# danieleschmidt/grid-fed-rl-gym

Hardware: AMD Instinct MI355X
Metric: env steps/sec (batched feeders) (higher is better)
Workload: dtype f64

## Files before the change

grid_fed_rl_gym_amd/csrc/abi_debug.hip:

```cpp
#include <cstdlib>
#include <cstring>
#include <string>
#include <vector>

#include "handle.h"
#include "mesh_schedule.h"

using namespace gsi;

extern "C" {

int gs_mesh_schedule_dump(const gs_topology* topo, int32_t zero_z_mode, int32_t nw, int32_t ni, int32_t acc_cap, int32_t unit_budget, int32_t region_base,
                          int32_t slot_bytes, int32_t* header, char* why, int32_t why_cap, void* items, int32_t* rowinfo,
                          int32_t* adj_off, double* adj_y) {
  if (!topo || !header) return fail(nullptr, GS_E_INVALID, "topology / header is NULL");
  if (topo->struct_size != (int32_t)sizeof(gs_topology)) return fail(nullptr, GS_E_INVALID, "struct_size mismatch");
  if (nw < 1 || ni < 1 || acc_cap < 1) return fail(nullptr, GS_E_INVALID, "bad arguments");
  HostTopology ht;
  const std::string err = gs_compile_topology(*topo, zero_z_mode, false, true, ht);
  if (!err.empty()) return fail(nullptr, GS_E_INVALID, "topology: %s", err.c_str());
  MeshSchedule S;
  gs_mesh_schedule(ht, nw, ni, 8, region_base, slot_bytes, acc_cap, unit_budget, S);
  const int32_t hd[16] = {S.ok ? 1 : 0, S.n_levels, S.n_rows, S.max_rows_per_wave, S.n_pivots, S.msg_units, S.n_messages, S.n_accumulators,
                          S.max_degree, S.unit_bytes, S.zero_off, S.dummy_off, S.body_off, S.region_bytes, (int32_t)sizeof(GsMeshItem), (int32_t)S.adj_off.size()};
// ... 18 lines not shown
  gs_mesh_schedule(ht, nw, ni, 8, region_base, slot_bytes, acc_cap, unit_budget, S);
  if (!S.ok) return fail(nullptr, GS_E_TOPOLOGY, "%s", S.why.c_str());
  counts[0] = S.n_pairs; counts[1] = (int32_t)S.ytab.size(); counts[2] = (int32_t)S.adj_ent.size(); counts[3] = GS_MESH_WORDS;
  if (packed) memcpy(packed, S.packed.data(), S.packed.size() * sizeof(int32_t));
  if (rowinfo) memcpy(rowinfo, S.rowinfo_packed.data(), S.rowinfo_packed.size() * sizeof(int32_t));
  if (ytab) memcpy(ytab, S.ytab.data(), S.ytab.size() * sizeof(double));
  if (adj_ent) memcpy(adj_ent, S.adj_ent.data(), S.adj_ent.size() * sizeof(int32_t));
  return GS_OK;
}

int gs_flat_newton_map_dump(const gs_topology* topo, int32_t zero_z_mode, double* out) {
  if (!topo || !out) return fail(nullptr, GS_E_INVALID, "topology / out is NULL");
  if (topo->struct_size != (int32_t)sizeof(gs_topology)) return fail(nullptr, GS_E_INVALID, "struct_size mismatch");
  HostTopology ht;
  const std::string err = gs_compile_topology(*topo, zero_z_mode, false, true, ht);
  if (!err.empty()) return fail(nullptr, GS_E_INVALID, "topology: %s", err.c_str());
  for (int i = 0; i < ht.n; ++i)
    if (i != ht.slack && !(ht.th_free[i] && ht.vm_free[i])) return fail(nullptr, GS_E_TOPOLOGY, "a bus other than the slack is not a PQ bus");
  const int na = ht.n - 1, N2 = 2 * na, K = na + 1, tiles = (N2 + 15) / 16, steps = (K + 3) / 4;
  std::vector<double> wt;
  if (!flat_newton_map(ht, tiles, steps, wt)) return fail(nullptr, GS_E_TOPOLOGY, "the flat-start Jacobian is singular");
  for (int u = 0; u < N2; ++u)
    for (int k = 0; k < K; ++k) out[(size_t)u * K + k] = wt[((size_t)(u / 16) * steps + k / 4) * 64 + (u % 16) + 16 * (k % 4)];
  return GS_OK;
}

int gs_debug_stamps(gs_handle* h, uint64_t* cycles_out, int32_t n) {
  if (!h || !cycles_out || n < 1 || n > 16) return fail(h, GS_E_INVALID, "bad arguments");
  GS_ENTER(h);
  HIPCHK(h, hipStreamSynchronize(h->stream));
  if (!h->d_stamps) {
    int rc = dev_alloc(h, &h->d_stamps, 16 + 2 * GS_STAMP_BLOCKS);
    if (rc) return rc;
    HIPCHK(h, hipMemset(h->d_stamps, 0, (16 + 2 * GS_STAMP_BLOCKS) * sizeof(unsigned long long)));
    h->SC.stamps = h->d_stamps;
    h->DA.stamps = h->d_stamps;
    h->SA.stamps = h->d_stamps;
    h->SC.stamp_wave = getenv("GS_STAMP_WAVE") ? atoi(getenv("GS_STAMP_WAVE")) : 0;
    h->SC.block_times = getenv("GS_STAMP_BLOCK_TIMES") ? 1 : 0;
    for (int k = 0; k < n; ++k) cycles_out[k] = 0;
    return GS_OK;
  }
  unsigned long long tmp[16];
  HIPCHK(h, hipMemcpy(tmp, h->d_stamps, sizeof tmp, hipMemcpyDeviceToHost));
  HIPCHK(h, hipMemset(h->d_stamps, 0, sizeof tmp));
  for (int k = 0; k < n; ++k) cycles_out[k] = tmp[k];
// ... 104 lines not shown
```

grid_fed_rl_gym_amd/csrc/gridstep_abi.hip:

```cpp
#include <hip/hip_runtime.h>

#include <algorithm>
#include <cmath>
#include <cstdarg>
#include <cstdio>
#include <cstdlib>
#include <cstring>
#include <string>
#include <vector>

#include "handle.h"

using namespace gsi;

namespace {

thread_local std::string g_last_error;

int launch_pack(gs_handle* h, const int32_t* map, int C, double* dst) {
  if (C <= 0) return GS_OK;
  LaunchTimer lt(h, GS_K_PACK);
  dim3 grid(h->groups, (C + 63) / 64);
  hipLaunchKernelGGL(gs_k_pack, grid, dim3(256), 0, h->stream, map, h->d_cst, C, h->R.total, h->slab, dst, h->B);
  HIPCHK(h, hipGetLastError());
// ... 387 lines not shown
  UP(lu_orig_pos, lu_orig_pos);
  if ((rc = dev_upload(h, &T.lu_a_ptr, h->lu_a_ptr)) || (rc = dev_upload(h, &T.lu_a, h->lu_a)) || (rc = dev_upload(h, &T.lu_b_ptr, h->lu_b_ptr)) ||
      (rc = dev_upload(h, &T.lu_b, h->lu_b)) || (rc = dev_upload(h, &T.lu_c_ptr, h->lu_c_ptr)) || (rc = dev_upload(h, &T.lu_c, h->lu_c)) ||
      (rc = dev_upload(h, &T.lu_r_ptr, h->lu_r_ptr)) || (rc = dev_upload(h, &T.lu_r, h->lu_r))) return bail(rc);
  UP(dn_th_idx, dn_th_idx); UP(dn_vm_idx, dn_vm_idx);
  UP(bl_ptr, bl_ptr); UP(bl_idx, bl_idx); UP(bg_ptr, bg_ptr); UP(bg_idx, bg_idx); UP(bb_ptr, bb_ptr); UP(bb_idx, bb_idx);
  UP(load_base, load_base); UP(load_q, load_q); UP(gen_kind, gen_kind); UP(gen_cap, gen_cap); UP(gen_p0, gen_p0);
  UP(gen_p1, gen_p1); UP(gen_p2, gen_p2); UP(bat_cap, bat_cap); UP(bat_rating, bat_rating); UP(bat_eff, bat_eff);
#undef UP
  if (h->solve == SolveMember::nr_dense_mfma) {
    GsDenseArgs& D = h->DA;
    if ((rc = dev_upload(h, &D.act_bus, h->act_bus)) || (rc = dev_upload(h, &D.act_of, h->act_of)) || (rc = dev_upload(h, &D.ent_ptr, h->ent_ptr)) ||
        (rc = dev_upload(h, &D.ent, h->ent)) || (rc = dev_upload(h, &D.bent_ptr, h->bent_ptr)) || (rc = dev_upload(h, &D.bent, h->bent))) return bail(rc);
    D.row_ptr = T.row_ptr; D.col = T.col; D.G = T.G; D.Bv = T.Bv; D.Gd = T.Gd; D.Bd = T.Bd;
    D.th_free = T.th_free; D.vm_free = T.vm_free; D.fixed_v = T.fixed_v; D.v_set = T.v_set;
    const size_t blocks = (size_t)D.NB * D.NB * 64 * 64;
    if ((rc = dev_alloc(h, &D.scratch, (size_t)h->dense_grid * blocks)) || (h->dense_flat && (rc = dev_alloc(h, &D.flat, blocks + 8))) ||
        (!h->jinv_t.empty() && (rc = dev_upload(h, &D.jinv_t, h->jinv_t)))) return bail(rc);
  }
  if (h->step == StepMember::nr_mesh2 &&
      ((rc = dev_upload(h, &h->F2.mesh_items, h->mesh_items)) || (rc = dev_upload(h, &h->F2.mesh_rowinfo, h->mesh_rowinfo)))) return bail(rc);
  if (h->second_gen() &&
      ((rc = dev_upload(h, &h->F2.recs, h->f2recs)) || (rc = dev_upload(h, &h->F2.anc, h->f2anc)) || (rc = dev_upload(h, &h->F2.zbus, h->f2z)) ||
       (h->fs_slot.size() > 1 && ((rc = dev_upload(h, &h->F2.fixed_slot, h->fs_slot)) || (rc = dev_upload(h, &h->F2.fixed_val, h->fs_val)))))) return bail(rc);
  if (h->pz) {
    GsLineParamArgs& A = h->LP;
    const size_t Bm = (size_t)h->B * h->m;
    h->inst_r.assign(topo->line_r_inst, topo->line_r_inst + Bm); h->inst_x.assign(topo->line_x_inst, topo->line_x_inst + Bm);
    A.B = h->B; A.groups = h->groups; A.n_slots = ht.n + 3; A.m = ht.m; A.newton = h->f2().newton() ? 1 : 0;
    A.lyr_nom = T.lyr; A.lyi_nom = T.lyi;
    double *dr = nullptr, *dx = nullptr, *dpz = nullptr;
    const size_t n_pz = (size_t)h->groups * GS_PZ_NQ(A.n_slots, A.m) * GS_LANES * 2;
    if ((rc = dev_upload(h, &A.zero_z, h->pz_zero)) || (rc = dev_upload(h, &A.ops_ptr, h->pz_ops_ptr)) || (rc = dev_upload(h, &A.ops, h->pz_ops)) ||
        (rc = dev_upload(h, &A.has, h->pz_has)) || (rc = dev_alloc(h, &dr, Bm)) || (rc = dev_alloc(h, &dx, Bm)) ||
        (rc = dev_alloc(h, &h->d_pzmask, (size_t)h->B)) || (rc = dev_alloc(h, &dpz, n_pz))) return bail(rc);
    A.r = dr; A.x = dx; A.pz = dpz;
    if (hipMemcpy(dr, h->inst_r.data(), Bm * sizeof(double), hipMemcpyHostToDevice) != hipSuccess ||
        hipMemcpy(dx, h->inst_x.data(), Bm * sizeof(double), hipMemcpyHostToDevice) != hipSuccess ||
        hipMemset(dpz, 0, n_pz * sizeof(double)) != hipSuccess || hipDeviceSynchronize() != hipSuccess)
      return bail(fail(nullptr, GS_E_HIP, "per-instance line impedances: upload failed"));
    if ((rc = launch_line_params(h, nullptr))) return bail(fail(nullptr, rc, "%s", h->err.c_str()));
  }
  if (h->pl) {
    GsLoadParamArgs& A = h->LL;
    const size_t Bl = (size_t)h->B * h->n_loads;
    h->inst_load.assign(topo->load_base_inst, topo->load_base_inst + Bl);
// ... 455 lines not shown
```

grid_fed_rl_gym_amd/csrc/gs_internal.h:

```cpp
#pragma once
#include <stdint.h>

#if defined(GS_BUILD_EXPERIMENTS)
#define GS_EXPERIMENT_ENV(name) getenv(name)
#else
#define GS_EXPERIMENT_ENV(name) ((const char*)nullptr)
#endif

#define GS_LANES 64
#define GS_ELEM(row, lane) ((((size_t)(row) >> 1) << 7) + ((size_t)(lane) << 1) + ((size_t)(row) & 1))
#define GS_MAX_WAVES 16
#define GS_ELL_K 4

#if defined(__HIP_DEVICE_COMPILE__)
#define GS_CONST __attribute__((address_space(4)))
#else
#define GS_CONST
#endif

#define GS_ARGS_IN_PLACE(Block, name)                                                                                           \
  const __attribute__((address_space(4))) char* ka_ = (const __attribute__((address_space(4))) char*)__builtin_amdgcn_kernarg_segment_ptr(); \
  asm volatile("" : "+s"(ka_));                                                                                                \
  const Block* name = (const Block*)ka_

// ... 250 lines not shown
  unsigned long long* stamps;
  GsRows R;
};

struct GsPackArgs {
  const int32_t* map;
  const double* cst;
  double* out;
  int32_t obs_dim, tiles_per_pass;
  int32_t early_pass0, pair_ok;
  int32_t skip0, skip1;
  int32_t lean, pad0;
};

#define GS_F2_PITCH 33
#define GS_F2_CHILDREN 8
struct GsF2Rec {
  int32_t bus, parent, flags, last;
  int32_t nl, l0, l1, ng;
  int32_t g0, g1, nb, b0;
  int32_t b1, level, pad1, pad2;
  double zr, zi, yr, yi;
};
#define GS_MESH_ACC 4
struct GsMeshItem {
  int32_t vk_off, vj_off;
  int32_t xk_off, xj_off;
  int32_t flags;
  int32_t cq_off;
  int32_t adj_ptr, bus;
  double ykj_g, ykj_b, ykk_g, ykk_b;
  int32_t mout[8];
  int32_t cq_in[GS_MESH_ACC], rw_in[GS_MESH_ACC], cl_in[GS_MESH_ACC];
  int32_t nbr, pos;
  int32_t pad[10];
};
enum {
  GS_MESH_F_PIVOT = 1,
  GS_MESH_F_NBR = 2,
  GS_MESH_F_SLACKPOS = 4,
  GS_MESH_F_HV0_SHIFT = 4,
  GS_MESH_F_T_SHIFT = 8,
  GS_MESH_F_G_SHIFT = 12,
  GS_MESH_F_RMW_SHIFT = 16
};

// ... 8 lines not shown
  GS_MESH_WORDS = 16
};
#define GS_MESH_F_NADJ_SHIFT 24

struct GsF2Tables {
  const GsF2Rec* recs;
  const int32_t* anc;
  const double* zbus;
  int32_t n_slots;
  int32_t slack;
  int32_t n_jump;
  int32_t n_levels, pos_off, n_anc_ints, wg_offset;
  int32_t off_tile, off_anc, off_z, off_env, off_red, off_atom, lds_bytes;
  int32_t off_prof, ring_zero;
  int32_t env_genp, env_curt, env_batp, env_soc;
  int32_t n_fixed, fixed_slot0;
  double fixed_val0;
  const int32_t* fixed_slot; const double* fixed_val;
  double* nrflat; int32_t nrflat_mode, pad_nrflat;
  const int32_t* mesh_items; const int32_t* mesh_rowinfo;
  int32_t off_scr, mesh_nz;
  int32_t mesh_pairs, mesh_off_p;
  const double* mesh_w; int32_t mesh_w_steps, mesh_slack;
};

struct GsRolloutPostArgs {
  double* rew; uint8_t* done;
  double* obs_next;
  const int32_t* map; const double* cst;
  int32_t* term_count; int32_t* term_idx; double* term_obs; int32_t term_cap;
  int32_t obs_dim, t, B;
};

struct GsRolloutStep {
  double* rew; uint8_t* done;
  double* obs_prev;
  const int32_t* map; const double* cst;
  int32_t* term_count; int32_t* term_idx; double* term_obs;
  int32_t term_cap, obs_dim, t, active;
};

#define GS_STAMP_BLOCKS 2048
struct GsSolveCfg {
  double tolerance, alpha;
  int32_t max_iterations, jacobian_exact;
  unsigned long long* stamps;
// ... 69 lines not shown
```

grid_fed_rl_gym_amd/csrc/kernels_flow2.hip:

```cpp
#include <hip/hip_runtime.h>
#include <math.h>
#include <limits.h>
#include <type_traits>
#include <utility>

#include "../../include/gridstep.h"
#include "gs_internal.h"
#include "kernels.h"
#include "members.h"

#define ROW(r) S[(size_t)(r) * GS_LANES]
#include "env_device.h"

#pragma clang fp contract(off)

extern __shared__ __attribute__((aligned(16))) char f2_lds[];

__device__ __forceinline__ void f2_sync() { asm volatile("s_waitcnt vmcnt(0) lgkmcnt(0)\n\ts_barrier" ::: "memory"); }
__device__ __forceinline__ void f2_lds_sync() { asm volatile("s_waitcnt lgkmcnt(0)\n\ts_barrier" ::: "memory"); }

#define F2_AS3 __attribute__((address_space(3)))
#define F2_P(type, off) ((type F2_AS3*)((F2_AS3 char*)f2_lds + (off)))
#define F2_VP(type, off) ((volatile type F2_AS3*)((F2_AS3 char*)f2_lds + (off)))
typedef double f2_v2 __attribute__((ext_vector_type(2)));
// ... 106 lines not shown
  if (!st.done) {
    st.mm = mm; st.iters = it + 1;
    if (!(mm < INFINITY)) { st.status = GS_STATUS_NAN; st.done = true; }
    else if (crit < tol) { st.conv = 1; st.status = GS_STATUS_OK; st.done = true; }
  }
}
#define F2_SUM_SCALE 0x1p44
__device__ __forceinline__ unsigned long long f2_fix(double s) {
  const double d = __builtin_fma(fmin(s, 255.0), F2_SUM_SCALE, 0x1p52);
  return __builtin_bit_cast(unsigned long long, d) & 0x000fffffffffffffull;
}
__device__ __forceinline__ unsigned long long f2_fix_tolerance(double tol) {
  const double t = fmin(fmax(tol, 0.0), 255.0) * (0.5 * F2_SUM_SCALE);
  return (unsigned long long)t;
}
__device__ __forceinline__ void f2_check_sum(F2State& st, double mm, unsigned long long sum_fix, unsigned long long tol_fix, int it) {
  if (!st.done) {
    st.mm = mm; st.iters = it + 1;
    if (!(mm < INFINITY)) { st.status = GS_STATUS_NAN; st.done = true; }
    else if (sum_fix < tol_fix) { st.conv = 1; st.status = GS_STATUS_OK; st.done = true; }
  }
}

__device__ __forceinline__ double f2_angle(double f, double e) {
  if (!__all(e > 0.0 && fabs(f) <= 0.125 * e)) return atan2(f, e);
  const double t = f / e, z = t * t;
  double p = -1.0 / 19.0;
  p = __builtin_fma(p, z, 1.0 / 17.0); p = __builtin_fma(p, z, -1.0 / 15.0); p = __builtin_fma(p, z, 1.0 / 13.0);
  p = __builtin_fma(p, z, -1.0 / 11.0); p = __builtin_fma(p, z, 1.0 / 9.0); p = __builtin_fma(p, z, -1.0 / 7.0);
  p = __builtin_fma(p, z, 1.0 / 5.0); p = __builtin_fma(p, z, -1.0 / 3.0);
  return __builtin_fma(t * z, p, t);
}

__device__ const double kF2Series[16] = {-1.0 / 355687428096000.0, 1.0 / 1307674368000.0, -1.0 / 6227020800.0, 1.0 / 39916800.0, -1.0 / 362880.0,
                                         1.0 / 5040.0, -1.0 / 120.0, 1.0 / 6.0,
                                         1.0 / 20922789888000.0, -1.0 / 87178291200.0, 1.0 / 479001600.0, -1.0 / 3628800.0, 1.0 / 40320.0,
                                         -1.0 / 720.0, 1.0 / 24.0, -0.5};
enum { F2_ST_PROLOGUE = 0, F2_ST_INIT, F2_ST_MISMATCH, F2_ST_BOTTOM_UP, F2_ST_FLAG, F2_ST_TOP_DOWN, F2_ST_FINAL_MISMATCH, F2_ST_EPILOGUE,
       F2_ST_PRO_SCALAR, F2_ST_PRO_SPARE, F2_ST_EPI_BUSES, F2_ST_EPI_LINES, F2_ST_EPI_REDUCE, F2_ST_EPI_SCALARS };
struct F2Stamp {
  unsigned long long* p; unsigned long long t; bool mine;
  __device__ __forceinline__ void hit(int k) {
    if (p == nullptr) return;
    const unsigned long long now = __builtin_readcyclecounter();
    if (mine) p[k] += now - t;
    t = now;
  }
};

template <int SOLVER, int CHK, int NW, int NI, int IW, int PZ = 0, int PL = 0>
__device__ __forceinline__ void f2_step(const GsTables& T, const GsF2Tables& F, const GsRows& R, const GsSolveCfg& C, const GsEnvCfg& E,
                                        double* __restrict__ slab, int B, const double* __restrict__ actions, double total_load,
                                        const GsPackArgs& PA, const GsFusedChecks& FC, const GsRolloutStep& RS,
                                        const double* __restrict__ pz = nullptr, const double* __restrict__ pl = nullptr) {
  f2_touch_arguments();
  constexpr int HV = 64 / IW;
  constexpr unsigned SB = (unsigned)(IW + 1) * 16u;
  const int lane = threadIdx.x & 63, l = lane & (IW - 1), hv = lane / IW;
  auto f2_slot = [](int slot, int ll) -> unsigned { return __umul24((unsigned)slot, SB) + ((unsigned)ll << 4); };
  const int wave = __builtin_amdgcn_readfirstlane(threadIdx.x >> 6);
  const int bid = (int)blockIdx.x + F.wg_offset;
  const int g = bid / HV, hs = bid % HV, L = hs * IW + l;
  const int b = g * GS_LANES + L;
  const bool valid = b < B;
  const GsLaneRows S = gs_lane_rows(slab, g, R.total, L);
  const double* const pz_lane = PZ ? pz + ((size_t)g * GS_PZ_NQ(F.n_slots, T.m) * GS_LANES + L) * 2 : nullptr;
  auto pz_at = [&](int q) -> double2 { return *(const double2*)(pz_lane + (size_t)q * (2 * GS_LANES)); };
  const double* const pl_lane = PL ? pl + ((size_t)g * GS_PL_NQ(T.n_loads) * GS_LANES + L) * 2 : nullptr;
  auto pl_at = [&](int q) -> double2 { return *(const double2*)(pl_lane + (size_t)q * (2 * GS_LANES)); };
  int n = T.n, m = T.m, nsl = F.n_slots;
  int o_env = F.off_env, o_tile = F.off_tile, o_red = F.off_red, o_atom = F.off_atom, o_anc = F.off_anc, o_z = F.off_z, o_prof = F.off_prof;
  int n_tab = SOLVER == F2_FBS ? F.n_jump * nsl * 4 : F.n_anc_ints;
  const int32_t* anc_g = F.anc; const double* zbus_g = F.zbus;
// ... 1025 lines not shown
    auto publish = [&]() {
#pragma unroll
      for (int j = 0; j < NI; ++j) f2_st2(bufA + f2_slot(ibus[j], l), make_double2(sr[j], si[j]));
    };
    const bool cap = it + 1 >= C.max_iterations;
    if (!cap) {
      unsigned long long sum;
      const double mm = wg_max_sum(lmax, lsum, sum);
      stp.hit(F2_ST_FLAG);
      f2_check_sum(st, mm, sum, tol_fix, it + 1);
    }
    if (cap || __all(st.done)) { publish(); break; }
    if (!st.done) {
#pragma unroll
      for (int j = 0; j < NI; ++j) {
        const double rd = f2_rcp(__builtin_fma(sr[j], sr[j], si[j] * si[j]));
        IR[j] = (Pj[j] * sr[j]) * rd; II[j] = (Pj[j] * si[j]) * rd;
      }
    }
    backward([]() -> bool { return false; });
    stp.hit(F2_ST_BOTTOM_UP);
  }
  }
  f2_sync();
  stp.hit(F2_ST_FINAL_MISMATCH);

  const bool flat_lane = st.done && st.iters <= 1, any_flat = __any(flat_lane);
  auto final_ef = [&](int bus) -> double2 {
    double2 v = f2_ld2(f2_slot(bus, l));
    if (any_flat) { const double fv = T.fixed_v[bus] ? T.v_set[bus] : 1.0; if (flat_lane) v = make_double2(fv, 0.0); }
    return v;
  };
  double totloss0 = 0.0, f_old = 0.0, viol0 = 0.0, step0 = 0.0, eprew0 = 0.0;
  if (wave == 0) { totloss0 = ROW(R.TOTLOSS); f_old = ROW(R.FREQ); viol0 = ROW(R.VIOL); eprew0 = ROW(R.EPREW); step0 = valid ? kold + 1.0 : kold; }
  const bool chk = CHK && FC.enabled;
  if (chk && wave == 0 && hv == 0) { cell[l] = 0ull; cell[IW + l] = 0ull; }
  const GsChecksCfg& K = FC.C;
  double* Pv = chk ? FC.prev + (size_t)g * (n + 1) * GS_LANES + L : nullptr;
  constexpr int BUS_PASSES = CHK ? NI + 1 : 1;
  double pvp[BUS_PASSES];
  double pv_f = 0.0;
  int ck_has_prev = 0, ck_consec = 0, ck_emode = 0;
  if constexpr (CHK) {
    if (chk) {
#pragma unroll
      for (int q = 0; q < BUS_PASSES; ++q) { const int i0 = wave * HV + hv + q * HV * NW; pvp[q] = i0 < n ? Pv[(size_t)i0 * GS_LANES] : 0.0; }
      if (wave == 0) pv_f = Pv[(size_t)n * GS_LANES];
      if (wave == 0 && hv == 0 && b < (int)FC.Bp && valid) { ck_has_prev = FC.state[b]; ck_consec = FC.state[FC.Bp + b]; ck_emode = FC.state[2 * FC.Bp + b]; }
    }
  }
  int k_nlow = 0, k_nhigh = 0, k_mhigh = 0, k_mlow = 0, k_mem = 0, k_cover = 0, k_mover = 0, k_vbad = 0, k_fbad = 0;
  double k_dv = 0.0, k_ql = 0.0; int k_dvnan = 0, k_qlnan = 0;

  int over = 0;
  for (int k0 = wave * HV + hv; k0 < ((m + HV * NW - 1) / (HV * NW)) * (HV * NW); k0 += HV * NW) {
    const bool on = k0 < m; const int k = on ? k0 : m - 1;
    const int li = T.lfrom[k], lj = T.lto[k];
    double yr, yi;
    if constexpr (PZ != 0) { const double2 y = pz_at(2 * nsl + k); yr = y.x; yi = y.y; } else { yr = T.lyr[k]; yi = T.lyi[k]; }
    const double rating = T.lrating[k], rinv = T.lrating_inv[k];
    const double2 vi = final_ef(li), vj = final_ef(lj);
    const double dr = vi.x - vj.x, di = vi.y - vj.y;
    const double ir = __builtin_fma(yr, dr, -(yi * di)), ii = __builtin_fma(yr, di, yi * dr);
    const double sr = __builtin_fma(vi.x, ir, vi.y * ii), si = __builtin_fma(vi.y, ir, -(vi.x * ii));
    const double ql = (rating > 0.0) ? gs_div_by(sqrt(__builtin_fma(sr, sr, si * si)), rating, rinv) : 0.0;
    const double ld = (rating > 0.0) ? gs_div_by(fabs(sr), rating, rinv) : 0.0;
    if (on) {
      f2_row(S, R.LOAD + k) = ql;
      if (!PA.lean) f2_pair(S, R.FLOW + k) = make_double2(sr, ld);
      f2_st2(o_tile + (unsigned)k * SB + ((unsigned)l << 4), make_double2(sr, ld));
      over += (ld > 0.8) ? 1 : 0;
      if (chk) {
        const double cld_ = K.stride_cload == 2 ? ld : ql;
        const bool co = cld_ > K.c_load, mo = cld_ > K.m_load;
        k_cover += co; k_mover += mo;
        if (ql != ql) k_qlnan = 1; else k_ql = fmax(k_ql, ql);
        if (!(fabs(sr) < INFINITY)) k_fbad = 1;
        if (FC.line_mask) FC.line_mask[((size_t)g * m + k) * GS_LANES + L] = (uint8_t)(co | (mo << 1));
      }
    }
  }
  stp.hit(F2_ST_EPI_LINES);
  f2_lds_sync();
  double dev = 0.0, vmax = -INFINITY, vmin = INFINITY;
  int vflags = 0;
  auto bus_pass = [&](int i0, double pv) {
    const bool on = i0 < n; const int i = on ? i0 : n - 1;
    double2 ef = final_ef(i);
    if (!on) ef = make_double2(1.0, 0.0);
    const double v = sqrt(__builtin_fma(ef.x, ef.x, ef.y * ef.y));
    const double ang = f2_angle(ef.y, ef.x);
    if (on) {
      f2_st2(f2_slot(i, l), make_double2(v, ang));
      if (!PA.lean) f2_pair(S, R.VM + i) = make_double2(v, ang);
      dev += fabs(v - 1.0);
      vmax = fmax(vmax, v); vmin = fmin(vmin, v);
      vflags |= (v > E.v_max) ? 1 : 0;
      vflags |= (v < E.v_min) ? 2 : 0;
      if (chk) {
        const bool cl = v < K.c_vlo, ch = !cl && v > K.c_vhi;
        const bool mh = v > K.m_vhi, ml = v < K.m_vlo;
        const bool em = v > K.m_evhi || v < K.m_evlo;
        k_nlow += cl; k_nhigh += ch; k_mhigh += mh; k_mlow += ml; k_mem += em;
        const double d = fabs(v - pv);
        if (d != d) k_dvnan = 1; else k_dv = fmax(k_dv, d);
        Pv[(size_t)i * GS_LANES] = v;
        if (!(fabs(v) < INFINITY)) k_vbad = 1;
        if (FC.bus_mask) FC.bus_mask[((size_t)g * n + i) * GS_LANES + L] = (uint8_t)(cl | (ch << 1) | (ml << 2) | (mh << 3) | (em << 4));
      }
    }
  };
  const int bus_passes = (n + HV * NW - 1) / (HV * NW);
  if constexpr (CHK) {
    if (chk) {
#pragma unroll
      for (int q = 0; q < BUS_PASSES; ++q) { if (q < bus_passes) bus_pass(wave * HV + hv + q * HV * NW, pvp[q]); }
    } else {
      for (int i0 = wave * HV + hv; i0 < bus_passes * (HV * NW); i0 += HV * NW) bus_pass(i0, 0.0);
    }
  } else {
    for (int i0 = wave * HV + hv; i0 < bus_passes * (HV * NW); i0 += HV * NW) {
      const bool on = i0 < n; const int i = on ? i0 : n - 1;
      double2 ef = final_ef(i);
      if (!on) ef = make_double2(1.0, 0.0);
      const double v = sqrt(__builtin_fma(ef.x, ef.x, ef.y * ef.y));
      const double ang = f2_angle(ef.y, ef.x);
      if (on) {
        f2_st2(f2_slot(i, l), make_double2(v, ang));
        if (!PA.lean) f2_pair(S, R.VM + i) = make_double2(v, ang);
        dev += fabs(v - 1.0);
        vmax = fmax(vmax, v); vmin = fmin(vmin, v);
        vflags |= (v > E.v_max) ? 1 : 0;
        vflags |= (v < E.v_min) ? 2 : 0;
      }
    }
  }
  stp.hit(F2_ST_EPI_BUSES);
  {
    const double ls2 = f2_xsum<IW>(psum, l), dv2 = f2_xsum<IW>(dev, l);
    if (hv == 0) { red_lsum[wave * IW + l] = ls2; red_dev[wave * IW + l] = dv2; }
    if (vmax == vmax && vmax > -INFINITY) atomicMax(cell + 3 * IW + l, f2_bits(vmax));
    if (vmin == vmin && vmin < INFINITY) atomicMin(cell + 4 * IW + l, f2_bits(vmin));
    if (over) atomicAdd(icell + 0 * IW + l, (unsigned)over);
    if (vflags) atomicOr(icell + 1 * IW + l, (unsigned)vflags);
    if (chk) {
      if (k_nlow) atomicAdd(icell + 2 * IW + l, (unsigned)k_nlow);
      if (k_nhigh) atomicAdd(icell + 3 * IW + l, (unsigned)k_nhigh);
      if (k_mhigh) atomicAdd(icell + 4 * IW + l, (unsigned)k_mhigh);
      if (k_mlow) atomicAdd(icell + 5 * IW + l, (unsigned)k_mlow);
      if (k_mem) atomicAdd(icell + 6 * IW + l, (unsigned)k_mem);
      if (k_cover) atomicAdd(icell + 7 * IW + l, (unsigned)k_cover);
      if (k_mover) atomicAdd(icell + 8 * IW + l, (unsigned)k_mover);
      const unsigned fl = (unsigned)(k_vbad | (k_fbad << 1) | (k_dvnan << 2) | (k_qlnan << 3));
      if (fl) atomicOr(icell + 9 * IW + l, fl);
      atomicMax(cell + 0 * IW + l, f2_bits(k_dv));
      atomicMax(cell + 1 * IW + l, f2_bits(k_ql));
    }
  }
  f2_lds_sync();
// ... 125 lines not shown
    if (st.mm > K.q_tol * 100.0) q *= 0.6;
    if (st.iters <= 5) q *= 1.1; else if (st.iters > 20) q *= 0.9;
    q = fmin(q, 1.0);
    if (!st.conv || vbad || fbad) q = 0.0;
    OF(GS_CF_QUALITY) = q;
#undef OI
#undef OF
  }
  stp.hit(F2_ST_EPI_SCALARS);
  if (C.stamps && C.block_times && lane == 0 && bid < GS_STAMP_BLOCKS)
    atomicMax(&C.stamps[17 + 2 * bid], (unsigned long long)__builtin_amdgcn_s_memrealtime());
}

template <StepMember M> constexpr GsStepKernels f2_kernels() { return {}; }
#define F2_PTR_0(p) nullptr
#define F2_PTR_1(p) p
#define F2_KERNEL(kernel, name, CHK, PZ, PL, OCC)                                                                           \
  extern "C" __global__ void __launch_bounds__(64 * step_row(StepMember::name).nw) OCC                                      \
  kernel(GsTables T, GsF2Tables F, GsRows R, GsSolveCfg C, GsEnvCfg E, double* __restrict__ slab, int B,                     \
         const double* __restrict__ actions, double total_load, GsPackArgs PA, GsFusedChecks FC, GsRolloutStep RS,          \
         const double* __restrict__ pz, const double* __restrict__ pl) {                                                    \
    constexpr StepMemberRow r = step_row(StepMember::name);                                                                 \
    GS_ARGS_IN_PLACE(F2ArgBlock, A);                                                                                        \
    f2_step<r.solver, CHK, r.nw, r.ni, r.iw, PZ, PL>(A->T, A->F, A->R, A->C, A->E, A->slab, A->B, A->actions, A->total_load, A->PA, \
                                                   A->FC, A->RS, F2_PTR_##PZ(pz), F2_PTR_##PL(pl));                         \
  }
#define F2_FORM(name, suffix, PZ, PL, OCC)                                                                                  \
  F2_KERNEL(gs_k_step_##name##suffix, name, 0, PZ, PL, OCC)                                                                 \
  F2_KERNEL(gs_k_stepc_##name##suffix, name, 1, PZ, PL, OCC)
#define F2_FNS(name, suffix) {gs_k_step_##name##suffix, gs_k_stepc_##name##suffix}
#define F2_MEMBER_NO_PZ(name, OCC)                                                                                          \
  F2_FORM(name, , 0, 0, OCC)                                                                                                \
  F2_FORM(name, _pl, 0, 1, OCC)                                                                                             \
  template <> constexpr GsStepKernels f2_kernels<StepMember::name>() { return {{{F2_FNS(name, ), F2_FNS(name, _pl)}, {}}}; }
#define F2_MEMBER(name, OCC)                                                                                                \
  F2_FORM(name, , 0, 0, OCC)                                                                                                \
  F2_FORM(name, _pl, 0, 1, OCC)                                                                                             \
  F2_FORM(name, _pz, 1, 0, OCC)                                                                                             \
  F2_FORM(name, _pz_pl, 1, 1, OCC)                                                                                          \
  template <> constexpr GsStepKernels f2_kernels<StepMember::name>() {                                                      \
    return {{{F2_FNS(name, ), F2_FNS(name, _pl)}, {F2_FNS(name, _pz), F2_FNS(name, _pz_pl)}}};                              \
  }

#if defined(GS_BUILD_EXPERIMENTS)
F2_MEMBER_NO_PZ(fbs_flow2, )
#endif
F2_MEMBER(nr_flow2, )
// ... 107 lines not shown
```

grid_fed_rl_gym_amd/csrc/members.h:

```cpp
#pragma once
#include <cstddef>

enum class SolveMember { nr_tree, nr_sparse_lu, fbs, nr_dense_pivot, nr_tree_lds, fbs_lds, fbs_flow, nr_dense_mfma, nr_sparse_lds };

enum class StepMember {
  none, fbs_flow2s, fbs_flow2h, fbs_flow2x,
#if defined(GS_BUILD_EXPERIMENTS)
  fbs_flow2,
#endif
  nr_flow2s, nr_flow2, nr_mesh2
};
constexpr int kStepMemberCount = (int)StepMember::nr_mesh2 + 1;

enum { F2_FBS = 0, F2_NR = 1, F2_NRM = 2 };

struct StepMemberRow {
  const char* name;
  int solver, nw, ni, iw;
  bool pz;
  constexpr int positions() const { return nw * (64 / iw) * ni; }
  constexpr bool newton() const { return solver == F2_NR || solver == F2_NRM; }
};
constexpr StepMemberRow kStepMembers[] = {
    {"none", -1, 0, 0, 64, false},
    {"fbs_flow2s", F2_FBS, 2, 1, 8, true},
    {"fbs_flow2h", F2_FBS, 8, 4, 16, true},
    {"fbs_flow2x", F2_FBS, 8, 8, 16, true},
#if defined(GS_BUILD_EXPERIMENTS)
    {"fbs_flow2", F2_FBS, 16, 4, 32, false},
#endif
    {"nr_flow2s", F2_NR, 4, 1, 8, true},
    {"nr_flow2", F2_NR, 8, 8, 32, true},
    {"nr_mesh2", F2_NRM, 4, 10, 8, false},
};
static_assert(sizeof kStepMembers / sizeof *kStepMembers == (size_t)kStepMemberCount, "one row per StepMember");
constexpr const StepMemberRow& step_row(StepMember s) { return kStepMembers[(int)s]; }
```

grid_fed_rl_gym_amd/csrc/plan.cpp:

```cpp
#include "plan.h"

#include <algorithm>
#include <cmath>
#include <cstdarg>
#include <cstdio>
#include <cstdlib>
#include <map>

#include "mesh_schedule.h"

namespace {

std::string reject(GsPlan& p, int code, const char* fmt, ...) {
  char buf[512];
  va_list ap; va_start(ap, fmt); vsnprintf(buf, sizeof buf, fmt, ap); va_end(ap);
  p.err_code = code;
  return buf;
}

const char* const kSolveName[] = {"nr_tree", "nr_sparse_lu", "fbs", "nr_dense_pivot", "nr_tree_lds", "fbs_lds", "fbs_flow", "nr_dense_mfma", "nr_sparse_lds"};
static_assert(sizeof kSolveName / sizeof *kSolveName == (size_t)SolveMember::nr_sparse_lds + 1, "kSolveName");

template <typename Rec>
void device_fields(const HostTopology& ht, int i, Rec& r) {
// ... 820 lines not shown
      return msg;
    }
  }
  return "";
}

std::string gs_plan(const gs_topology& topo, const gs_config& cfg, const HostTopology& ht, int batch, int cus, GsPlan& p) {
  p.B = batch; p.Bp = (batch + 63) / 64 * 64; p.groups = p.Bp / 64;
  int W = cfg.waves_per_group;
  if (const char* e = getenv("GS_WAVES")) W = atoi(e);
  const bool auto_w = W <= 0;
  if (W <= 0) { W = 1; while (W < 16 && p.groups * W * 2 <= 2048) W *= 2; }
  p.W = std::min(W, GS_MAX_WAVES);
  std::string why = plan_solve(cfg, ht, auto_w, p);
  if (!why.empty()) return why;
  p.dyn_lds = std::max<size_t>(49152 + 2 * 64 * 65 * sizeof(double), p.dyn_lds);
  p.n = ht.n; p.m = ht.m; p.n_loads = topo.n_loads; p.n_gens = topo.n_gens; p.n_bats = topo.n_bats;
  p.obs_dim = 2 * p.n + 2 * p.m + 1 + 2 * p.n_loads + p.n_gens + 2 * p.n_bats;
  p.action_dim = p.n_bats + p.n_gens;
  p.state_dim = 12 + 2 * p.n_bats + p.n_gens + 2 * p.n + 2 * p.m;
  plan_rows(ht, p);
  plan_work_lists(ht, p);
  plan_second_gen(topo, cfg, ht, auto_w, p);
  p.pz = topo.line_r_inst != nullptr;
  p.nr_flat = p.f2().newton() && !getenv("GS_NR_NO_FLAT") && !p.pz;
  if (p.pz && (why = plan_line_params(topo, cfg, ht, p)).empty() == false) { p.err_code = GS_E_TOPOLOGY; return why; }
  p.pl = topo.load_base_inst != nullptr;
  if (p.pl && (why = plan_load_params(topo, cfg, ht, p)).empty() == false) { p.err_code = GS_E_TOPOLOGY; return why; }
  if (ht.has_lu) plan_lu_schedule(ht, p);
  if (p.solve == SolveMember::nr_dense_mfma && !(why = plan_dense(cfg, ht, cus, p)).empty()) return why;
#if defined(GS_BUILD_EXPERIMENTS)
  if (p.solve == SolveMember::nr_sparse_lds && !(why = plan_sparse_lds(cfg, ht, cus, p)).empty()) return why;
#endif
  p.lean = p.second_gen() && !getenv("GS_EAGER_ROWS");
  p.split_ok = p.second_gen() && 2 * (size_t)p.F2.lds_bytes <= 160 * 1024 && !getenv("GS_NO_SPLIT") && p.groups * (64 / p.f2().iw) >= 512 &&
               p.groups >= 2;
  p.SC.tolerance = cfg.tolerance; p.SC.alpha = cfg.acceleration_factor;
  p.SC.max_iterations = cfg.max_iterations; p.SC.jacobian_exact = (cfg.jacobian_mode == GS_JACOBIAN_EXACT);
  GsEnvCfg& E = p.EC;
  E.timestep = cfg.timestep; E.v_min = cfg.v_min; E.v_max = cfg.v_max; E.f_min = cfg.f_min; E.f_max = cfg.f_max;
  E.safety_penalty = cfg.safety_penalty; E.H = cfg.inertia_H; E.D = cfg.damping_D; E.f0 = cfg.f_nominal;
  E.power_base = cfg.power_base; E.inv_power_base = 1.0 / cfg.power_base; E.episode_length = cfg.episode_length; E.stochastic_loads = cfg.stochastic_loads;
  E.fbs_warm_start = cfg.fbs_warm_start; E.weather_variation = cfg.weather_variation;
  p.total_load = 0.0;
  for (int l = 0; l < p.n_loads; ++l) p.total_load += topo.load_base[l];
  return plan_maps(ht, p);
}

void gs_plan_format(const GsPlan& p, const HostTopology& ht, char* buf, int buflen) {
  const bool f2 = p.second_gen(), dense = p.solve == SolveMember::nr_dense_mfma;
  snprintf(buf, buflen,
           "{\"kernel\": \"%s\", \"n\": %d, \"m\": %d, \"nnz\": %d, \"forest\": %s, \"levels\": %d, \"max_level_width\": %d, "
           "\"lu_slots\": %d, \"lu_orig\": %d, \"lu_pairs\": %lld, \"waves_per_group\": %d, \"groups\": %d, "
           "\"rows_per_group\": %d, \"slab_bytes\": %zu, \"obs_dim\": %d, \"action_dim\": %d, "
           "\"instances_per_workgroup\": %d, \"workgroups\": %d, \"step_lds_bytes\": %zu, \"step_launches\": %d, \"solve_kernel\": \"%s\", \"flow2\": \"%s\", "
           "\"mesh2\": \"%s\", \"mesh_levels\": %d, \"mesh_rows\": %d, \"mesh_message_units\": %d, \"mesh_messages\": %d, \"mesh_accumulators\": %d, "
           "\"dense_form\": \"%s\", \"dense_workgroups\": %d, \"dense_lds_bytes\": %zu, \"per_instance_z\": %d, \"nr_flat_start_table\": %d, "
           "\"per_instance_loads\": %d}",
           f2 ? p.f2().name : kSolveName[(int)p.solve], p.n, p.m, ht.nnz, ht.is_forest ? "true" : "false", ht.n_levels,
           ht.max_level_width, ht.lu_n_slots, ht.lu_n_orig, (long long)ht.lu_n_pairs, f2 ? p.f2().nw : p.W, p.groups,
           p.R.total, (size_t)p.groups * p.R.total * GS_LANES * sizeof(double), p.obs_dim, p.action_dim,
           f2 ? p.f2().iw : 64, f2 ? (64 / p.f2().iw) * p.groups : p.groups, f2 ? (size_t)p.F2.lds_bytes : p.dyn_lds + 24576, p.split_ok ? 2 : 1,
           kSolveName[(int)p.solve], f2 ? "on" : (p.flow2_why.empty() ? "n/a" : p.flow2_why.c_str()),
           p.step == StepMember::nr_mesh2 ? "on" : (p.mesh_why.empty() ? "n/a" : p.mesh_why.c_str()), p.mesh_levels, p.mesh_rows, p.mesh_units,
           p.mesh_messages, p.mesh_accs, dense ? (p.dense_blockrow ? "block_row" : "panel") : "n/a", dense ? p.dense_grid : 0, dense ? p.dense_lds : (size_t)0,
           p.pz ? 1 : 0, p.nr_flat ? 1 : 0, p.pl ? 1 : 0);
}
```

grid_fed_rl_gym_amd/csrc/plan.h:

```cpp
#pragma once
#include <cstddef>
#include <cstdint>
#include <string>
#include <vector>

#include "../../include/gridstep.h"
#include "gs_internal.h"
#include "members.h"
#include "topology.h"

enum { SF_REWARD = 0, SF_VMAX, SF_VMIN, SF_LOSSES, SF_EPREW, SF_MAXMIS, SF_COUNT };
enum { SI_VIOL = 0, SI_STEP, SI_ITERS, SI_STATUS, SI_COUNT };
enum { SU_TERM = 0, SU_TRUNC, SU_CONV, SU_VF0, SU_VF1, SU_VF2, SU_VF3, SU_COUNT };

struct GsPlan {
  int err_code = 0;
  SolveMember solve = SolveMember::fbs;
  StepMember step = StepMember::none;
  int B = 0, Bp = 0, groups = 0, W = 1;
  int n = 0, m = 0, obs_dim = 0, action_dim = 0, state_dim = 0;
  int n_loads = 0, n_gens = 0, n_bats = 0;
  size_t dyn_lds = 0;
  GsRows R{};
  GsSolveCfg SC{};
  GsEnvCfg EC{};
  double total_load = 0.0;
  GsF2Tables F2{};
  std::string flow2_why, mesh_why;
  int mesh_levels = 0, mesh_rows = 0, mesh_units = 0, mesh_messages = 0, mesh_accs = 0;
  GsDenseArgs DA{}; int dense_grid = 0; size_t dense_lds = 0; bool dense_blockrow = true, dense_flat = false;
  GsSparseArgs SA{}; int sparse_grid = 0; size_t sparse_lds = 0;
  bool split_ok = false, lean = false;
  int obs_skip0 = 0, obs_skip1 = 0;

  std::vector<GsItemRec> witems; std::vector<int32_t> wl_ptr, ovf_slot;
  std::vector<GsInjRec> winj; std::vector<int32_t> wi_ptr;
  std::vector<GsBusRec> wbus; std::vector<int32_t> wb_ptr;
  std::vector<GsF2Rec> f2recs; std::vector<int32_t> f2anc; std::vector<double> f2z;
  std::vector<int32_t> fs_slot; std::vector<double> fs_val;
  std::vector<double> mesh_w;
  std::vector<int32_t> mesh_items, mesh_rowinfo;
  std::vector<int32_t> lu_a_ptr, lu_a, lu_b_ptr, lu_b, lu_c_ptr, lu_c, lu_r_ptr, lu_r;
  std::vector<int32_t> act_bus, act_of, ent_ptr, ent, bent_ptr; std::vector<GsDenseEntry> bent;
  std::vector<double> jinv_t;
  std::vector<int32_t> mo, mvm, mva, mfl, mld, mp, mq, mact, mst; std::vector<double> cst;
  std::vector<int32_t> rf, ri, ru;
#if defined(GS_BUILD_EXPERIMENTS)
  std::vector<int32_t> ipack; std::vector<double> dpack;
#endif

  bool pz = false, nr_flat = false;
  std::vector<int32_t> pz_ops_ptr, pz_ops; std::vector<uint8_t> pz_has, pz_zero;

  bool pl = false;
  std::vector<double> pl_tan;

  bool second_gen() const { return step != StepMember::none; }
  const StepMemberRow& f2() const { return step_row(step); }
};

std::string gs_plan(const gs_topology& topo, const gs_config& cfg, const HostTopology& ht, int batch, int cus, GsPlan& out);
std::string gs_check_line_impedances(const gs_topology& topo, int batch, const double* r_inst, const double* x_inst, const uint8_t* mask);
std::string gs_check_load_powers(int n_loads, int batch, const double* base_inst, const uint8_t* mask);
void gs_plan_format(const GsPlan& p, const HostTopology& ht, char* buf, int buflen);
bool flat_newton_map(const HostTopology& ht, int tiles, int steps, std::vector<double>& wt);
```

Baseline: 261.6 million.

## Pack line records into 48-byte structs, prefetch ahead, specialize bus-angle series

Packs each line's endpoints, admittance and rating into one aligned 48-byte record uploaded at plan time. FBS step members then load the first record before the final barrier and prefetch the next record while the current line is processed, replacing six scattered table loads. The bus epilogue also gets a fast path that checks the small-angle condition per pass and uses the arctangent series with coefficients loaded from constant memory, falling back to the general path otherwise. This adds a device table, more template variants and more registers per kernel.

Measured after the change: 263.8 million (median of 6 runs). About the same (+0.9%).

```diff
diff --git a/grid_fed_rl_gym_amd/csrc/abi_debug.hip b/grid_fed_rl_gym_amd/csrc/abi_debug.hip
--- a/grid_fed_rl_gym_amd/csrc/abi_debug.hip
+++ b/grid_fed_rl_gym_amd/csrc/abi_debug.hip
@@ -64,6 +64,18 @@
   if (!flat_newton_map(ht, tiles, steps, wt)) return fail(nullptr, GS_E_TOPOLOGY, "the flat-start Jacobian is singular");
   for (int u = 0; u < N2; ++u)
     for (int k = 0; k < K; ++k) out[(size_t)u * K + k] = wt[((size_t)(u / 16) * steps + k / 4) * 64 + (u % 16) + 16 * (k % 4)];
+  return GS_OK;
+}
+
+int gs_line_records_dump(const gs_topology* topo, int32_t zero_z_mode, void* out, int32_t record_bytes) {
+  if (!topo || !out) return fail(nullptr, GS_E_INVALID, "topology / out is NULL");
+  if (topo->struct_size != (int32_t)sizeof(gs_topology)) return fail(nullptr, GS_E_INVALID, "struct_size mismatch");
+  if (record_bytes != (int32_t)sizeof(GsF2LineRec)) return fail(nullptr, GS_E_INVALID, "a line record is %d bytes", (int)sizeof(GsF2LineRec));
+  HostTopology ht;
+  const std::string err = gs_compile_topology(*topo, zero_z_mode, false, true, ht);
+  if (!err.empty()) return fail(nullptr, GS_E_INVALID, "topology: %s", err.c_str());
+  const std::vector<GsF2LineRec> recs = gs_line_records(ht);
+  if (!recs.empty()) memcpy(out, recs.data(), recs.size() * sizeof(GsF2LineRec));
   return GS_OK;
 }
 
diff --git a/grid_fed_rl_gym_amd/csrc/gridstep_abi.hip b/grid_fed_rl_gym_amd/csrc/gridstep_abi.hip
--- a/grid_fed_rl_gym_amd/csrc/gridstep_abi.hip
+++ b/grid_fed_rl_gym_amd/csrc/gridstep_abi.hip
@@ -433,6 +433,7 @@
       ((rc = dev_upload(h, &h->F2.mesh_items, h->mesh_items)) || (rc = dev_upload(h, &h->F2.mesh_rowinfo, h->mesh_rowinfo)))) return bail(rc);
   if (h->second_gen() &&
       ((rc = dev_upload(h, &h->F2.recs, h->f2recs)) || (rc = dev_upload(h, &h->F2.anc, h->f2anc)) || (rc = dev_upload(h, &h->F2.zbus, h->f2z)) ||
+       (rc = dev_upload(h, &h->F2.lines, h->f2lines)) ||
        (h->fs_slot.size() > 1 && ((rc = dev_upload(h, &h->F2.fixed_slot, h->fs_slot)) || (rc = dev_upload(h, &h->F2.fixed_val, h->fs_val)))))) return bail(rc);
   if (h->pz) {
     GsLineParamArgs& A = h->LP;
diff --git a/grid_fed_rl_gym_amd/csrc/gs_internal.h b/grid_fed_rl_gym_amd/csrc/gs_internal.h
--- a/grid_fed_rl_gym_amd/csrc/gs_internal.h
+++ b/grid_fed_rl_gym_amd/csrc/gs_internal.h
@@ -296,6 +296,12 @@
   int32_t b1, level, pad1, pad2;
   double zr, zi, yr, yi;
 };
+struct alignas(16) GsF2LineRec {
+  int32_t from, to, pad[2];
+  double yr, yi;
+  double rating, rating_inv;
+};
+static_assert(sizeof(GsF2LineRec) == 48, "three 16-byte loads per line record");
 #define GS_MESH_ACC 4
 struct GsMeshItem {
   int32_t vk_off, vj_off;
@@ -350,6 +356,7 @@
   int32_t off_scr, mesh_nz;
   int32_t mesh_pairs, mesh_off_p;
   const double* mesh_w; int32_t mesh_w_steps, mesh_slack;
+  const GsF2LineRec* lines;
 };
 
 struct GsRolloutPostArgs {
diff --git a/grid_fed_rl_gym_amd/csrc/kernels_flow2.hip b/grid_fed_rl_gym_amd/csrc/kernels_flow2.hip
--- a/grid_fed_rl_gym_amd/csrc/kernels_flow2.hip
+++ b/grid_fed_rl_gym_amd/csrc/kernels_flow2.hip
@@ -152,13 +152,31 @@
   }
 }
 
+__device__ __forceinline__ bool f2_angle_near(double f, double e) { return __all(e > 0.0 && fabs(f) <= 0.125 * e); }
 __device__ __forceinline__ double f2_angle(double f, double e) {
-  if (!__all(e > 0.0 && fabs(f) <= 0.125 * e)) return atan2(f, e);
+  if (!f2_angle_near(f, e)) return atan2(f, e);
   const double t = f / e, z = t * t;
   double p = -1.0 / 19.0;
   p = __builtin_fma(p, z, 1.0 / 17.0); p = __builtin_fma(p, z, -1.0 / 15.0); p = __builtin_fma(p, z, 1.0 / 13.0);
   p = __builtin_fma(p, z, -1.0 / 11.0); p = __builtin_fma(p, z, 1.0 / 9.0); p = __builtin_fma(p, z, -1.0 / 7.0);
   p = __builtin_fma(p, z, 1.0 / 5.0); p = __builtin_fma(p, z, -1.0 / 3.0);
+  return __builtin_fma(t * z, p, t);
+}
+__device__ const double kF2Angle[9] = {-1.0 / 19.0, 1.0 / 17.0, -1.0 / 15.0, 1.0 / 13.0, -1.0 / 11.0, 1.0 / 9.0, -1.0 / 7.0, 1.0 / 5.0, -1.0 / 3.0};
+struct F2AngleCoef { double c[9]; };
+__device__ __forceinline__ F2AngleCoef f2_angle_coef() {
+  F2AngleCoef K;
+  const GS_CONST double* k0 = (const GS_CONST double*)kF2Angle;
+#pragma unroll
+  for (int q = 0; q < 9; ++q) K.c[q] = k0[q];
+  return K;
+}
+__device__ __forceinline__ double f2_angle_series(double f, double e, const F2AngleCoef& K) {
+  const double t = f / e, z = t * t;
+  double p = K.c[0];
+  p = __builtin_fma(p, z, K.c[1]); p = __builtin_fma(p, z, K.c[2]); p = __builtin_fma(p, z, K.c[3]);
+  p = __builtin_fma(p, z, K.c[4]); p = __builtin_fma(p, z, K.c[5]); p = __builtin_fma(p, z, K.c[6]);
+  p = __builtin_fma(p, z, K.c[7]); p = __builtin_fma(p, z, K.c[8]);
   return __builtin_fma(t * z, p, t);
 }
 
@@ -178,7 +196,7 @@
   }
 };
 
-template <int SOLVER, int CHK, int NW, int NI, int IW, int PZ = 0, int PL = 0>
+template <int SOLVER, int CHK, int NW, int NI, int IW, int PZ = 0, int PL = 0, int LA = -1>
 __device__ __forceinline__ void f2_step(const GsTables& T, const GsF2Tables& F, const GsRows& R, const GsSolveCfg& C, const GsEnvCfg& E,
                                         double* __restrict__ slab, int B, const double* __restrict__ actions, double total_load,
                                         const GsPackArgs& PA, const GsFusedChecks& FC, const GsRolloutStep& RS,
@@ -1250,7 +1268,24 @@
     stp.hit(F2_ST_BOTTOM_UP);
   }
   }
-  f2_sync();
+  struct F2Line { f2_i4 ft; f2_v2 y, rt; };
+  const int line0 = wave * HV + hv, line_end = ((m + HV * NW - 1) / (HV * NW)) * (HV * NW);
+  auto line_rec = [&](int k0) -> F2Line {
+    const char* const q = (const char*)(F.lines + (k0 < m ? k0 : m - 1));
+    F2Line r;
+    r.ft = *(const f2_i4*)q;
+    if constexpr (PZ != 0) { r.y.x = 0.0; r.y.y = 0.0; } else r.y = *(const f2_v2*)(q + 16);
+    r.rt = *(const f2_v2*)(q + 32);
+    return r;
+  };
+  F2Line line_cur{};
+  if constexpr (LA > 0) {
+    asm volatile("s_waitcnt vmcnt(0)" ::: "memory");
+    line_cur = line_rec(line0);
+    f2_lds_sync();
+  } else {
+    f2_sync();
+  }
   stp.hit(F2_ST_FINAL_MISMATCH);
 
   const bool flat_lane = st.done && st.iters <= 1, any_flat = __any(flat_lane);
@@ -1281,43 +1316,89 @@
   double k_dv = 0.0, k_ql = 0.0; int k_dvnan = 0, k_qlnan = 0;
 
   int over = 0;
-  for (int k0 = wave * HV + hv; k0 < ((m + HV * NW - 1) / (HV * NW)) * (HV * NW); k0 += HV * NW) {
-    const bool on = k0 < m; const int k = on ? k0 : m - 1;
-    const int li = T.lfrom[k], lj = T.lto[k];
-    double yr, yi;
-    if constexpr (PZ != 0) { const double2 y = pz_at(2 * nsl + k); yr = y.x; yi = y.y; } else { yr = T.lyr[k]; yi = T.lyi[k]; }
-    const double rating = T.lrating[k], rinv = T.lrating_inv[k];
-    const double2 vi = final_ef(li), vj = final_ef(lj);
-    const double dr = vi.x - vj.x, di = vi.y - vj.y;
-    const double ir = __builtin_fma(yr, dr, -(yi * di)), ii = __builtin_fma(yr, di, yi * dr);
-    const double sr = __builtin_fma(vi.x, ir, vi.y * ii), si = __builtin_fma(vi.y, ir, -(vi.x * ii));
-    const double ql = (rating > 0.0) ? gs_div_by(sqrt(__builtin_fma(sr, sr, si * si)), rating, rinv) : 0.0;
-    const double ld = (rating > 0.0) ? gs_div_by(fabs(sr), rating, rinv) : 0.0;
-    if (on) {
-      f2_row(S, R.LOAD + k) = ql;
-      if (!PA.lean) f2_pair(S, R.FLOW + k) = make_double2(sr, ld);
-      f2_st2(o_tile + (unsigned)k * SB + ((unsigned)l << 4), make_double2(sr, ld));
-      over += (ld > 0.8) ? 1 : 0;
-      if (chk) {
-        const double cld_ = K.stride_cload == 2 ? ld : ql;
-        const bool co = cld_ > K.c_load, mo = cld_ > K.m_load;
-        k_cover += co; k_mover += mo;
-        if (ql != ql) k_qlnan = 1; else k_ql = fmax(k_ql, ql);
-        if (!(fabs(sr) < INFINITY)) k_fbad = 1;
-        if (FC.line_mask) FC.line_mask[((size_t)g * m + k) * GS_LANES + L] = (uint8_t)(co | (mo << 1));
+  if constexpr (LA < 0) {
+    for (int k0 = wave * HV + hv; k0 < ((m + HV * NW - 1) / (HV * NW)) * (HV * NW); k0 += HV * NW) {
+      const bool on = k0 < m; const int k = on ? k0 : m - 1;
+      const int li = T.lfrom[k], lj = T.lto[k];
+      double yr, yi;
+      if constexpr (PZ != 0) { const double2 y = pz_at(2 * nsl + k); yr = y.x; yi = y.y; } else { yr = T.lyr[k]; yi = T.lyi[k]; }
+      const double rating = T.lrating[k], rinv = T.lrating_inv[k];
+      const double2 vi = final_ef(li), vj = final_ef(lj);
+      const double dr = vi.x - vj.x, di = vi.y - vj.y;
+      const double ir = __builtin_fma(yr, dr, -(yi * di)), ii = __builtin_fma(yr, di, yi * dr);
+      const double sr = __builtin_fma(vi.x, ir, vi.y * ii), si = __builtin_fma(vi.y, ir, -(vi.x * ii));
+      const double ql = (rating > 0.0) ? gs_div_by(sqrt(__builtin_fma(sr, sr, si * si)), rating, rinv) : 0.0;
+      const double ld = (rating > 0.0) ? gs_div_by(fabs(sr), rating, rinv) : 0.0;
+      if (on) {
+        f2_row(S, R.LOAD + k) = ql;
+        if (!PA.lean) f2_pair(S, R.FLOW + k) = make_double2(sr, ld);
+        f2_st2(o_tile + (unsigned)k * SB + ((unsigned)l << 4), make_double2(sr, ld));
+        over += (ld > 0.8) ? 1 : 0;
+        if (chk) {
+          const double cld_ = K.stride_cload == 2 ? ld : ql;
+          const bool co = cld_ > K.c_load, mo = cld_ > K.m_load;
+          k_cover += co; k_mover += mo;
+          if (ql != ql) k_qlnan = 1; else k_ql = fmax(k_ql, ql);
+          if (!(fabs(sr) < INFINITY)) k_fbad = 1;
+          if (FC.line_mask) FC.line_mask[((size_t)g * m + k) * GS_LANES + L] = (uint8_t)(co | (mo << 1));
+        }
+      }
+    }
+  } else {
+    auto line_pass = [&](int k0, const F2Line* rec) {
+      const bool on = k0 < m; const int k = on ? k0 : m - 1;
+      const int li = rec->ft.x, lj = rec->ft.y;
+      double yr, yi;
+      if constexpr (PZ != 0) { const double2 y = pz_at(2 * nsl + k); yr = y.x; yi = y.y; } else { yr = rec->y.x; yi = rec->y.y; }
+      const double rating = rec->rt.x, rinv = rec->rt.y;
+      const double2 vi = final_ef(li), vj = final_ef(lj);
+      const double dr = vi.x - vj.x, di = vi.y - vj.y;
+      const double ir = __builtin_fma(yr, dr, -(yi * di)), ii = __builtin_fma(yr, di, yi * dr);
+      const double sr = __builtin_fma(vi.x, ir, vi.y * ii), si = __builtin_fma(vi.y, ir, -(vi.x * ii));
+      const double ql = (rating > 0.0) ? gs_div_by(sqrt(__builtin_fma(sr, sr, si * si)), rating, rinv) : 0.0;
+      const double ld = (rating > 0.0) ? gs_div_by(fabs(sr), rating, rinv) : 0.0;
+      if (on) {
+        f2_row(S, R.LOAD + k) = ql;
+        if (!PA.lean) f2_pair(S, R.FLOW + k) = make_double2(sr, ld);
+        f2_st2(o_tile + (unsigned)k * SB + ((unsigned)l << 4), make_double2(sr, ld));
+        over += (ld > 0.8) ? 1 : 0;
+        if (chk) {
+          const double cld_ = K.stride_cload == 2 ? ld : ql;
+          const bool co = cld_ > K.c_load, mo = cld_ > K.m_load;
+          k_cover += co; k_mover += mo;
+          if (ql != ql) k_qlnan = 1; else k_ql = fmax(k_ql, ql);
+          if (!(fabs(sr) < INFINITY)) k_fbad = 1;
+          if (FC.line_mask) FC.line_mask[((size_t)g * m + k) * GS_LANES + L] = (uint8_t)(co | (mo << 1));
+        }
+      }
+    };
+    for (int k0 = line0; k0 < line_end; k0 += HV * NW) {
+      if constexpr (LA > 0) {
+        const F2Line nxt = line_rec(k0 + HV * NW);
+        line_pass(k0, &line_cur);
+        line_cur = nxt;
+      } else {
+        const F2Line rec = line_rec(k0);
+        line_pass(k0, &rec);
       }
     }
   }
   stp.hit(F2_ST_EPI_LINES);
+  const F2AngleCoef AK0 = f2_angle_coef();
   f2_lds_sync();
+  F2AngleCoef AK = AK0;
+#pragma unroll
+  for (int q = 0; q < 9; ++q) F2_KEEP(AK.c[q]);
   double dev = 0.0, vmax = -INFINITY, vmin = INFINITY;
   int vflags = 0;
-  auto bus_pass = [&](int i0, double pv) {
+  auto bus_pass = [&](int i0, double pv, auto near) -> bool {
     const bool on = i0 < n; const int i = on ? i0 : n - 1;
     double2 ef = final_ef(i);
     if (!on) ef = make_double2(1.0, 0.0);
+    if constexpr (decltype(near)::value) { if (!f2_angle_near(ef.y, ef.x)) return false; }
     const double v = sqrt(__builtin_fma(ef.x, ef.x, ef.y * ef.y));
-    const double ang = f2_angle(ef.y, ef.x);
+    double ang;
+    if constexpr (decltype(near)::value) ang = f2_angle_series(ef.y, ef.x, AK); else ang = f2_angle(ef.y, ef.x);
     if (on) {
       f2_st2(f2_slot(i, l), make_double2(v, ang));
       if (!PA.lean) f2_pair(S, R.VM + i) = make_double2(v, ang);
@@ -1337,22 +1418,26 @@
         if (FC.bus_mask) FC.bus_mask[((size_t)g * n + i) * GS_LANES + L] = (uint8_t)(cl | (ch << 1) | (ml << 2) | (mh << 3) | (em << 4));
       }
     }
+    return true;
   };
-  const int bus_passes = (n + HV * NW - 1) / (HV * NW);
+  const int bus_passes = (n + HV * NW - 1) / (HV * NW), bus_end = bus_passes * (HV * NW);
+  int i0 = wave * HV + hv;
   if constexpr (CHK) {
     if (chk) {
 #pragma unroll
-      for (int q = 0; q < BUS_PASSES; ++q) { if (q < bus_passes) bus_pass(wave * HV + hv + q * HV * NW, pvp[q]); }
+      for (int q = 0; q < BUS_PASSES; ++q) { if (q < bus_passes) bus_pass(i0 + q * HV * NW, pvp[q], std::false_type{}); }
+      i0 = bus_end;
     } else {
-      for (int i0 = wave * HV + hv; i0 < bus_passes * (HV * NW); i0 += HV * NW) bus_pass(i0, 0.0);
+      for (; i0 < bus_end; i0 += HV * NW) { if (!bus_pass(i0, 0.0, std::true_type{})) break; }
     }
   } else {
-    for (int i0 = wave * HV + hv; i0 < bus_passes * (HV * NW); i0 += HV * NW) {
+    for (; i0 < bus_end; i0 += HV * NW) {
       const bool on = i0 < n; const int i = on ? i0 : n - 1;
       double2 ef = final_ef(i);
       if (!on) ef = make_double2(1.0, 0.0);
+      if (!f2_angle_near(ef.y, ef.x)) break;
       const double v = sqrt(__builtin_fma(ef.x, ef.x, ef.y * ef.y));
-      const double ang = f2_angle(ef.y, ef.x);
+      const double ang = f2_angle_series(ef.y, ef.x, AK);
       if (on) {
         f2_st2(f2_slot(i, l), make_double2(v, ang));
         if (!PA.lean) f2_pair(S, R.VM + i) = make_double2(v, ang);
@@ -1363,6 +1448,7 @@
       }
     }
   }
+  for (; i0 < bus_end; i0 += HV * NW) bus_pass(i0, 0.0, std::false_type{});
   stp.hit(F2_ST_EPI_BUSES);
   {
     const double ls2 = f2_xsum<IW>(psum, l), dv2 = f2_xsum<IW>(dev, l);
@@ -1534,7 +1620,7 @@
          const double* __restrict__ pz, const double* __restrict__ pl) {                                                    \
     constexpr StepMemberRow r = step_row(StepMember::name);                                                                 \
     GS_ARGS_IN_PLACE(F2ArgBlock, A);                                                                                        \
-    f2_step<r.solver, CHK, r.nw, r.ni, r.iw, PZ, PL>(A->T, A->F, A->R, A->C, A->E, A->slab, A->B, A->actions, A->total_load, A->PA, \
+    f2_step<r.solver, CHK, r.nw, r.ni, r.iw, PZ, PL, r.line_ahead>(A->T, A->F, A->R, A->C, A->E, A->slab, A->B, A->actions, A->total_load, A->PA, \
                                                    A->FC, A->RS, F2_PTR_##PZ(pz), F2_PTR_##PL(pl));                         \
   }
 #define F2_FORM(name, suffix, PZ, PL, OCC)                                                                                  \
diff --git a/grid_fed_rl_gym_amd/csrc/members.h b/grid_fed_rl_gym_amd/csrc/members.h
--- a/grid_fed_rl_gym_amd/csrc/members.h
+++ b/grid_fed_rl_gym_amd/csrc/members.h
@@ -18,20 +18,21 @@
   const char* name;
   int solver, nw, ni, iw;
   bool pz;
+  int line_ahead;
   constexpr int positions() const { return nw * (64 / iw) * ni; }
   constexpr bool newton() const { return solver == F2_NR || solver == F2_NRM; }
 };
 constexpr StepMemberRow kStepMembers[] = {
-    {"none", -1, 0, 0, 64, false},
-    {"fbs_flow2s", F2_FBS, 2, 1, 8, true},
-    {"fbs_flow2h", F2_FBS, 8, 4, 16, true},
-    {"fbs_flow2x", F2_FBS, 8, 8, 16, true},
+    {"none", -1, 0, 0, 64, false, -1},
+    {"fbs_flow2s", F2_FBS, 2, 1, 8, true, 1},
+    {"fbs_flow2h", F2_FBS, 8, 4, 16, true, 1},
+    {"fbs_flow2x", F2_FBS, 8, 8, 16, true, 1},
 #if defined(GS_BUILD_EXPERIMENTS)
-    {"fbs_flow2", F2_FBS, 16, 4, 32, false},
+    {"fbs_flow2", F2_FBS, 16, 4, 32, false, 1},
 #endif
-    {"nr_flow2s", F2_NR, 4, 1, 8, true},
-    {"nr_flow2", F2_NR, 8, 8, 32, true},
-    {"nr_mesh2", F2_NRM, 4, 10, 8, false},
+    {"nr_flow2s", F2_NR, 4, 1, 8, true, -1},
+    {"nr_flow2", F2_NR, 8, 8, 32, true, -1},
+    {"nr_mesh2", F2_NRM, 4, 10, 8, false, -1},
 };
 static_assert(sizeof kStepMembers / sizeof *kStepMembers == (size_t)kStepMemberCount, "one row per StepMember");
 constexpr const StepMemberRow& step_row(StepMember s) { return kStepMembers[(int)s]; }
diff --git a/grid_fed_rl_gym_amd/csrc/plan.cpp b/grid_fed_rl_gym_amd/csrc/plan.cpp
--- a/grid_fed_rl_gym_amd/csrc/plan.cpp
+++ b/grid_fed_rl_gym_amd/csrc/plan.cpp
@@ -866,6 +866,7 @@
   plan_rows(ht, p);
   plan_work_lists(ht, p);
   plan_second_gen(topo, cfg, ht, auto_w, p);
+  if (p.second_gen()) p.f2lines = gs_line_records(ht);
   p.pz = topo.line_r_inst != nullptr;
   p.nr_flat = p.f2().newton() && !getenv("GS_NR_NO_FLAT") && !p.pz;
   if (p.pz && (why = plan_line_params(topo, cfg, ht, p)).empty() == false) { p.err_code = GS_E_TOPOLOGY; return why; }
@@ -891,6 +892,16 @@
   return plan_maps(ht, p);
 }
 
+std::vector<GsF2LineRec> gs_line_records(const HostTopology& ht) {
+  std::vector<GsF2LineRec> recs((size_t)ht.m, GsF2LineRec{});
+  for (int k = 0; k < ht.m; ++k) {
+    GsF2LineRec& r = recs[k];
+    r.from = ht.lfrom[k]; r.to = ht.lto[k];
+    r.yr = ht.lyr[k]; r.yi = ht.lyi[k]; r.rating = ht.lrating[k]; r.rating_inv = ht.lrating_inv[k];
+  }
+  return recs;
+}
+
 void gs_plan_format(const GsPlan& p, const HostTopology& ht, char* buf, int buflen) {
   const bool f2 = p.second_gen(), dense = p.solve == SolveMember::nr_dense_mfma;
   snprintf(buf, buflen,
diff --git a/grid_fed_rl_gym_amd/csrc/plan.h b/grid_fed_rl_gym_amd/csrc/plan.h
--- a/grid_fed_rl_gym_amd/csrc/plan.h
+++ b/grid_fed_rl_gym_amd/csrc/plan.h
@@ -38,6 +38,7 @@
   std::vector<GsBusRec> wbus; std::vector<int32_t> wb_ptr;
   std::vector<GsF2Rec> f2recs; std::vector<int32_t> f2anc; std::vector<double> f2z;
   std::vector<int32_t> fs_slot; std::vector<double> fs_val;
+  std::vector<GsF2LineRec> f2lines;
   std::vector<double> mesh_w;
   std::vector<int32_t> mesh_items, mesh_rowinfo;
   std::vector<int32_t> lu_a_ptr, lu_a, lu_b_ptr, lu_b, lu_c_ptr, lu_c, lu_r_ptr, lu_r;
@@ -63,4 +64,5 @@
 std::string gs_check_line_impedances(const gs_topology& topo, int batch, const double* r_inst, const double* x_inst, const uint8_t* mask);
 std::string gs_check_load_powers(int n_loads, int batch, const double* base_inst, const uint8_t* mask);
 void gs_plan_format(const GsPlan& p, const HostTopology& ht, char* buf, int buflen);
+std::vector<GsF2LineRec> gs_line_records(const HostTopology& ht);
 bool flat_newton_map(const HostTopology& ht, int tiles, int steps, std::vector<double>& wt);
```
